# staple/spark-agd

Measured on NVIDIA H100. Metric: AGD examples/sec (rows x applySmooth passes / s), logistic 10M x 1024 dense fp32, higher is better.
Workload: dtype f64

## Files before the change

spark-agd_b200/csrc/k1_tc.cu:

```cuda
#include <cuda.h>
#include <cuda_bf16.h>
#include <cuda_runtime.h>
#include <stdint.h>

#include "agd_common.cuh"
#include "k1_device.cuh"

namespace agd {

namespace {

constexpr int kKR = 16;
constexpr int kRegsConsumer = 64, kRegsAux = 56, kRegsMma = 168;
constexpr int kBlockBytes = kKR * 128;
constexpr int kBBytes = 1024;
constexpr int kScaleOff = 768;

__device__ __forceinline__ uint32_t smem_u32(const void *p) { return (uint32_t)__cvta_generic_to_shared(p); }
__device__ __forceinline__ void mbar_init(uint32_t bar, uint32_t count) {
  asm volatile("mbarrier.init.shared::cta.b64 [%0], %1;" ::"r"(bar), "r"(count));
}
__device__ __forceinline__ void mbar_expect_tx(uint32_t bar, uint32_t bytes) {
  asm volatile("mbarrier.arrive.expect_tx.shared::cta.b64 _, [%0], %1;" ::"r"(bar), "r"(bytes) : "memory");
}
__device__ __forceinline__ void mbar_arrive(uint32_t bar) {
  asm volatile("mbarrier.arrive.shared::cta.b64 _, [%0];" ::"r"(bar) : "memory");
}
__device__ __forceinline__ void mbar_wait(uint32_t bar, uint32_t parity) {
  asm volatile(
      "{\n\t.reg .pred p;\n\t"
      "WAIT_LOOP:\n\t"
      "mbarrier.try_wait.parity.shared::cta.b64 p, [%0], %1;\n\t"
      "@p bra WAIT_DONE;\n\t"
      "bra WAIT_LOOP;\n\t"
      "WAIT_DONE:\n\t}" ::"r"(bar),
      "r"(parity)
      : "memory");
}
__device__ __forceinline__ void named_arrive(int id, int count) {
// ... 1 lines not shown
}
__device__ __forceinline__ void named_sync(int id, int count) {
  asm volatile("bar.sync %0, %1;" ::"r"(id), "r"(count) : "memory");
}
__device__ __forceinline__ void tma_bulk_g2s(uint32_t dst, const void *src, uint32_t bytes, uint32_t bar) {
  asm volatile("cp.async.bulk.shared::cluster.global.mbarrier::complete_tx::bytes [%0], [%1], %2, [%3];" ::"r"(dst),
               "l"(src), "r"(bytes), "r"(bar)
               : "memory");
}
__device__ __forceinline__ void tma_tile_2d(uint32_t dst, const CUtensorMap *map, int c0, int c1, uint32_t bar) {
  asm volatile("cp.async.bulk.tensor.2d.shared::cluster.global.mbarrier::complete_tx::bytes [%0], [%1, {%2, %3}], [%4];" ::"r"(dst),
               "l"(map), "r"(c0), "r"(c1), "r"(bar)
               : "memory");
}
__device__ __forceinline__ void tma_tile_3d(uint32_t dst, const CUtensorMap *map, int c0, int c1, int c2, uint32_t bar) {
  asm volatile("cp.async.bulk.tensor.3d.shared::cluster.global.mbarrier::complete_tx::bytes [%0], [%1, {%2, %3, %4}], [%5];" ::"r"(dst),
               "l"(map), "r"(c0), "r"(c1), "r"(c2), "r"(bar)
               : "memory");
}
__device__ __forceinline__ uint64_t gmma_desc(uint32_t addr, uint32_t lbo, uint32_t sbo, uint64_t layout) {
  return (uint64_t)((addr & 0x3FFFF) >> 4) | ((uint64_t)(lbo >> 4) << 16) | ((uint64_t)(sbo >> 4) << 32) | (layout << 62);
}
__device__ __forceinline__ void wgmma_fence() { asm volatile("wgmma.fence.sync.aligned;" ::: "memory"); }
__device__ __forceinline__ void wgmma_commit() { asm volatile("wgmma.commit_group.sync.aligned;" ::: "memory"); }
template <int N>
__device__ __forceinline__ void wgmma_wait() { asm volatile("wgmma.wait_group.sync.aligned %0;" ::"n"(N) : "memory"); }
template <int N>
__device__ __forceinline__ void wgmma_bf16(float (&d)[N / 2], uint64_t adesc, uint64_t bdesc);
template <>
__device__ __forceinline__ void wgmma_bf16<16>(float (&d)[8], uint64_t adesc, uint64_t bdesc) {
  asm volatile("{ .reg .pred p; setp.ne.b32 p, 0, 0;\n\t"
               "wgmma.mma_async.sync.aligned.m64n16k16.f32.bf16.bf16 {%0,%1,%2,%3,%4,%5,%6,%7}, %8, %9, p, 1, 1, 1, 0; }"
               : "+f"(d[0]), "+f"(d[1]), "+f"(d[2]), "+f"(d[3]), "+f"(d[4]), "+f"(d[5]), "+f"(d[6]), "+f"(d[7])
               : "l"(adesc), "l"(bdesc)
               : "memory");
}
template <>
__device__ __forceinline__ void wgmma_bf16<24>(float (&d)[12], uint64_t adesc, uint64_t bdesc) {
  asm volatile("{ .reg .pred p; setp.ne.b32 p, 0, 0;\n\t"
               "wgmma.mma_async.sync.aligned.m64n24k16.f32.bf16.bf16 {%0,%1,%2,%3,%4,%5,%6,%7,%8,%9,%10,%11}, %12, %13, p, 1, 1, 1, 0; }"
               : "+f"(d[0]), "+f"(d[1]), "+f"(d[2]), "+f"(d[3]), "+f"(d[4]), "+f"(d[5]), "+f"(d[6]), "+f"(d[7]),
                 "+f"(d[8]), "+f"(d[9]), "+f"(d[10]), "+f"(d[11])
               : "l"(adesc), "l"(bdesc)
               : "memory");
}

template <int N, bool TWO>
__device__ __forceinline__ void mma_accumulate(const float (&e)[2][N / 2], int hb, int hs, const double (&sc)[2], double &g,
                                               double *g2) {
  float v[6];
#pragma unroll
  for (int t = 0; t < (TWO ? 6 : 3); ++t) {
    const int i = t == 0 ? 0 : t == 1 ? 1 : t == 2 ? 4 : t == 3 ? 5 : t == 4 ? 8 : 9;
    const float x0 = hs ? e[0][i + 2] : e[0][i], x1 = hs ? e[1][i + 2] : e[1][i];
    v[t] = hb ? x1 : x0;
  }
  g += (((double)v[0] + (double)v[1]) + (double)v[2]) * sc[0];
  if (TWO) *g2 += (((double)v[3] + (double)v[4]) + (double)v[5]) * sc[1];
}
__device__ __forceinline__ double pow2i(int k) { return __longlong_as_double((long long)(k + 1023) << 52); }
__device__ __forceinline__ void mma_release(uint32_t empty_bar, int lane) {
  __syncwarp();
  if (lane == 0) mbar_arrive(empty_bar);
}

struct TcLayout {
  uint32_t ring_off, w_off, b2_off, partial_off, bars_off, g2_off, total;
};
__host__ __device__ inline TcLayout tc_layout(int ring_groups, int group_bytes, int d, bool two_gradient) {
  TcLayout L;
  L.ring_off = 0;
  L.w_off = (uint32_t)ring_groups * group_bytes;
  L.b2_off = L.w_off + (uint32_t)d * 8;
  L.partial_off = L.b2_off + 2 * kBBytes;
  L.bars_off = L.partial_off + 2 * kKR * 16 * 8;
  L.g2_off = L.bars_off + (2 * (uint32_t)ring_groups + 8) * 8;
  L.total = L.g2_off + (two_gradient ? (uint32_t)d * 8 : 0u);
  return L;
}

struct TcArgs {
  const double *labels;
  const double *w;
  const double *w2;
  double *slabs;
  long long rows;
  int d, kind, slab_stride;
  unsigned long long sample_seed, sample_thresh;
  long long row_base;
  const RowFilter *filt;
  const uint32_t *view_bits;
  int gb;
  int ngt;
  int ring_groups;
  int one_copy;
  int diag;
};

__host__ __device__ constexpr int tc_consumers(int rpt) { return rpt == 4 ? 256 : 512; }
__device__ __forceinline__ unsigned long long ffma2(unsigned long long a, unsigned long long b, unsigned long long c) {
  const float x = __fmaf_rn(__uint_as_float((uint32_t)a), __uint_as_float((uint32_t)b), __uint_as_float((uint32_t)c));
  const float y = __fmaf_rn(__uint_as_float((uint32_t)(a >> 32)), __uint_as_float((uint32_t)(b >> 32)),
                            __uint_as_float((uint32_t)(c >> 32)));
  return ((unsigned long long)__float_as_uint(y) << 32) | __float_as_uint(x);
}
__device__ __forceinline__ unsigned long long pack2(uint32_t lo, uint32_t hi) {
  unsigned long long d;
  asm("mov.b64 %0, {%1, %2};" : "=l"(d) : "r"(lo), "r"(hi));
  return d;
}

template <int RPT, bool F32, int DUAL, bool VIEW, bool BIAS>
__global__ void __launch_bounds__(tc_consumers(RPT) + 256, 1)
k1_tc_kernel(const __grid_constant__ CUtensorMap tmap, const __grid_constant__ CUtensorMap tmap3, const TcArgs a,
             const long long ntiles) {
  constexpr int kConsumers = tc_consumers(RPT);
  constexpr int kThreads = kConsumers + 256;
  constexpr int kN = DUAL == 2 ? 24 : 16;
  constexpr int kCW = kConsumers / 32;
  constexpr bool kRepartition = RPT != 4;
  extern __shared__ __align__(1024) unsigned char smem[];
  const int group_bytes = a.gb * kBlockBytes;
  const TcLayout L = tc_layout(a.ring_groups, group_bytes, a.d, DUAL == 2);
  double *w_s = reinterpret_cast<double *>(smem + L.w_off);
  unsigned char *b2 = smem + L.b2_off;
  double *partial = reinterpret_cast<double *>(smem + L.partial_off);
  const uint32_t bars = smem_u32(smem + L.bars_off);
  const int RG = a.ring_groups;
  const uint32_t wbar = bars + 16u * RG, b2_full = wbar + 8, b2_empty = b2_full + 16;
  const int tid = threadIdx.x, warp = tid >> 5, lane = tid & 31;
  const long long my_tiles = (ntiles - blockIdx.x + gridDim.x - 1) / gridDim.x;
  const int npairs = a.d / 128;
  double *slab = a.slabs + (size_t)blockIdx.x * a.slab_stride;

  if (tid == 0) {
    for (int g = 0; g < RG; ++g) {
      mbar_init(bars + 8u * g, 1);
      mbar_init(bars + 8u * (RG + g), 4);
    }
    mbar_init(wbar, 1);
    mbar_init(b2_full, 1); mbar_init(b2_full + 8, 1);
    mbar_init(b2_empty, 4); mbar_init(b2_empty + 8, 4);
    asm volatile("fence.mbarrier_init.release.cluster;" ::: "memory");
  }
  for (int i = tid; i < 2 * kBBytes / 4; i += kThreads) reinterpret_cast<uint32_t *>(b2)[i] = 0u;
  asm volatile("fence.proxy.async.shared::cta;" ::: "memory");
  __syncthreads();

  if (warp >= kCW && warp < kCW + 4) {
   if (kRepartition) asm volatile("setmaxnreg.dec.sync.aligned.u32 %0;" ::"n"(kRegsAux));
   if (warp == kCW) {
    if (lane == 0) {
      mbar_expect_tx(wbar, (uint32_t)a.d * 8u);
      tma_bulk_g2s(smem_u32(w_s), a.w, (uint32_t)a.d * 8u, wbar);
      int slot = -1;
      uint32_t epar = 0;
      bool wrapped = false;
      for (long long k = 0; k < my_tiles; ++k) {
        const long long row0 = (blockIdx.x + k * (long long)gridDim.x) * kKR;
        for (int gi = 0; gi < a.ngt; ++gi) {
          if (++slot == RG) { slot = 0; if (wrapped) epar ^= 1u; wrapped = true; }
          if (wrapped) mbar_wait(bars + 8u * (RG + slot), epar);
          const uint32_t full = bars + 8u * slot;
          mbar_expect_tx(full, (uint32_t)group_bytes);
          if (a.one_copy) {
            tma_tile_3d(smem_u32(smem + (size_t)slot * group_bytes), &tmap3, 0, (int)row0, gi * a.gb, full);
          } else {
            for (int b = 0; b < a.gb; ++b)
              tma_tile_2d(smem_u32(smem + (size_t)slot * group_bytes + b * kBlockBytes), &tmap, (gi * a.gb + b) * 64, (int)row0, full);
          }
        }
      }
    }
   } else if (warp == kCW + 2) {
    double lossacc = 0.0, cntacc = 0.0, multacc = 0.0;
    double ynext = 0.0;
    const int srow = lane & 15;
    const bool second = DUAL && lane >= kKR;
    if (lane < kKR || DUAL) {
      const long long r = (long long)blockIdx.x * kKR + srow;
      if (r < a.rows) ynext = a.labels[r];
    }
    const double *partial2 = partial + 2 * kKR * 2;
    for (long long k = 0; k < my_tiles; ++k) {
      const int bb = (int)(k & 1);
      const long long tile = blockIdx.x + k * (long long)gridDim.x;
      const long long left = a.rows - tile * kKR;
      const int rv = left < kKR ? (int)left : kKR;
      const double ylab = ynext;
      if (lane < kKR || DUAL) {
        const long long r = (tile + gridDim.x) * kKR + srow;
        if (r < a.rows) ynext = a.labels[r];
      }
      named_sync(1 + bb, kConsumers + 32);
      double mult = 0.0;
      bool nonfinite = false;
      if (lane < kKR || second) {
        double m;
        if (RPT) {
          const double *pp = second ? partial2 : partial;
          m = pp[(bb * kKR + srow) * 2] + pp[(bb * kKR + srow) * 2 + 1];
        } else {
          const double *pp = partial + (bb * kKR + lane) * 16;
          m = (((pp[0] + pp[1]) + (pp[2] + pp[3])) + ((pp[4] + pp[5]) + (pp[6] + pp[7]))) +
              (((pp[8] + pp[9]) + (pp[10] + pp[11])) + ((pp[12] + pp[13]) + (pp[14] + pp[15])));
        }
        if (BIAS) m += ld_volatile_f64(second ? a.w2 + a.d : a.w + a.d);
        nonfinite = (lane < kKR || DUAL == 2) && srow < rv && !isfinite(m);
        double mu, loss;
        loss_eval(a.kind, m, ylab, mu, loss);
        if (srow < rv && (!VIEW || ((a.view_bits[(tile * kKR + srow) >> 5] >> ((tile * kKR + srow) & 31)) & 1u) != 0u) &&
            row_selected(a.sample_seed, a.sample_thresh, a.row_base + tile * kKR + srow)) {
          mult = mu; lossacc += loss; cntacc += 1.0;
          if (BIAS) multacc += mu;
        }
      }
      named_arrive(3 + bb, kConsumers + 32);
      const uint32_t hw = (uint32_t)__double2hiint(mult) & 0x7fffffffu;
      const uint32_t hwf = hw | (nonfinite ? 0x80000000u : 0u);
      uint32_t top = __reduce_max_sync(0xffffffffu, lane < kKR ? hwf : 0u), top2 = 0u;
      if (DUAL == 2) top2 = __reduce_max_sync(0xffffffffu, lane < kKR ? 0u : hwf);
      if ((top | top2) >> 31) {
        top = __reduce_max_sync(0xffffffffu, lane < kKR ? hw : 0u);
        if (DUAL == 2) top2 = __reduce_max_sync(0xffffffffu, lane < kKR ? 0u : hw);
        const uint32_t fl = __ballot_sync(0xffffffffu, nonfinite && mult == 0.0);
        const uint32_t zero_rows = DUAL == 2 ? (fl & (fl >> 16) & 0xffffu) : fl;
        const int slot0 = (int)((k * a.ngt) % RG);
#pragma unroll 1
        for (uint32_t rows = zero_rows; rows; rows &= rows - 1u) {
          const int zr = __ffs(rows) - 1;
          int sl = slot0;
#pragma unroll 1
          for (int gi = 0; gi < a.ngt; ++gi) {
#pragma unroll 1
            for (int c = lane; c < a.gb * 8; c += 32)
              *reinterpret_cast<uint4 *>(smem + sl * group_bytes + (c >> 3) * kBlockBytes + zr * 128 + (c & 7) * 16) =
                  make_uint4(0u, 0u, 0u, 0u);
            if (++sl == RG) sl = 0;
          }
        }
      }
      uint32_t E = top >> 20;
      if (DUAL == 2 && second) E = top2 >> 20;
      const int s = E == 0x7ffu ? 0 : E == 0u ? -1022 : E == 0x7feu ? 1023 : (int)E - 1022;
      const int ns = -s;
      const double ms = (mult * pow2i(ns >> 1)) * pow2i(ns - (ns >> 1));
      if (k >= 2) mbar_wait(b2_empty + 8u * bb, (uint32_t)(((k >> 1) - 1) & 1));
      if (srow == 0 && (lane < kKR || (DUAL == 2 && second))) {
        reinterpret_cast<double *>(b2 + bb * kBBytes + kScaleOff)[second ? 1 : 0] = pow2i(s);
      }
      if (lane < kKR || (DUAL == 2 && second)) {
        const __nv_bfloat16 hi = __double2bfloat16(ms);
        const double r1 = ms - (double)__bfloat162float(hi);
        const __nv_bfloat16 mid = __double2bfloat16(r1);
        const double r2 = r1 - (double)__bfloat162float(mid);
        const __nv_bfloat16 lo = __double2bfloat16(r2);
        const int n0 = second ? 9 : 0, n1 = second ? 16 : 1, n2 = second ? 17 : 8;
        unsigned char *base = b2 + bb * kBBytes + (srow / 8) * 128 + (srow % 8) * 2;
#pragma unroll
        for (int t = 0; t < 4; ++t) {
          const int c0 = n0 + 2 * t, c1 = n1 + 2 * t, c2 = n2 + 2 * t;
          *reinterpret_cast<__nv_bfloat16 *>(base + (c0 / 8) * 256 + (c0 % 8) * 16) = hi;
          *reinterpret_cast<__nv_bfloat16 *>(base + (c1 / 8) * 256 + (c1 % 8) * 16) = mid;
          *reinterpret_cast<__nv_bfloat16 *>(base + (c2 / 8) * 256 + (c2 % 8) * 16) = lo;
        }
      }
      asm volatile("fence.proxy.async.shared::cta;" ::: "memory");
      __syncwarp();
      if (lane == 0) mbar_arrive(b2_full + 8u * bb);
    }
    for (int off = DUAL ? 8 : 16; off >= 1; off >>= 1) {
      lossacc += __shfl_xor_sync(0xffffffffu, lossacc, off);
      cntacc += __shfl_xor_sync(0xffffffffu, cntacc, off);
      if (BIAS) multacc += __shfl_xor_sync(0xffffffffu, multacc, off);
    }
    const int DB = a.d + (BIAS ? 1 : 0);
    if (lane == 0) {
      if (BIAS) slab[a.d] = multacc;
      slab[DB] = lossacc; slab[DB + 1] = cntacc; if (!DUAL) { slab[DB + 2] = 0.0; slab[DB + 3] = 0.0; }
    }
    if (DUAL && lane == kKR) {
      slab[DB + 2] = lossacc; slab[DB + 3] = cntacc;
      if (DUAL == 2) {
        double *slab2 = slab + DB + 4;
        if (BIAS) slab2[a.d] = multacc;
        slab2[DB] = lossacc; slab2[DB + 1] = cntacc; slab2[DB + 2] = 0.0; slab2[DB + 3] = 0.0;
      }
    }
   }
  } else if (warp >= kCW + 4) {
    if (kRepartition) asm volatile("setmaxnreg.inc.sync.aligned.u32 %0;" ::"n"(kRegsMma));
    const int mw = warp - (kCW + 4);
    const int q = lane >> 2, j = lane & 3;
    const int hb = j >> 1, hs = j & 1;
    const int fo = 64 * hb + 16 * mw + q + 8 * hs;
    double gacc[32];
#pragma unroll
    for (int p = 0; p < 32; ++p) gacc[p] = 0.0;
    double *g2 = reinterpret_cast<double *>(smem + L.g2_off);
    if (DUAL == 2)
      for (int p = 0; p < npairs; ++p) g2[128 * p + fo] = 0.0;
    const int hp = a.gb / 2;
    int slot = -1;
    uint32_t par = 1;
    float acc[2][kN / 2];
    for (long long k = 0; k < my_tiles; ++k) {
      const int bb = (int)(k & 1);
      mbar_wait(b2_full + 8u * bb, (uint32_t)((k >> 1) & 1));
      const uint64_t bdesc = gmma_desc(smem_u32(b2 + bb * kBBytes), 128, 256, 0);
      const double *scs = reinterpret_cast<const double *>(b2 + bb * kBBytes + kScaleOff);
      const double sc[2] = {scs[0], DUAL == 2 ? scs[1] : 1.0};
#pragma unroll
      for (int p = 0; p < 32; ++p) {
        if (p < npairs) {
          const int pg = p % hp;
          if (pg == 0) {
            if (++slot == RG) slot = 0;
            if (slot == 0) par ^= 1u;
            mbar_wait(bars + 8u * slot, par);
          }
          const uint32_t a0 = smem_u32(smem + (size_t)slot * group_bytes + (2 * pg) * kBlockBytes);
          wgmma_fence();
          if (a.diag != 101) {
            wgmma_bf16<kN>(acc[0], gmma_desc(a0, kBlockBytes, 1024, 1), bdesc);
            wgmma_bf16<kN>(acc[1], gmma_desc(a0 + kBlockBytes, kBlockBytes, 1024, 1), bdesc);
          }
          wgmma_commit();
          wgmma_wait<0>();
          mma_accumulate<kN, DUAL == 2>(acc, hb, hs, sc, gacc[p], g2 + 128 * p + fo);
          if (pg == hp - 1) mma_release(bars + 8u * (RG + slot), lane);
        }
      }
      __syncwarp();
      if (lane == 0) mbar_arrive(b2_empty + 8u * bb);
    }
#pragma unroll
    for (int p = 0; p < 32; ++p)
      if (p < npairs) {
        slab[128 * p + fo] = gacc[p];
        if (DUAL == 2) slab[a.d + (BIAS ? 1 : 0) + 4 + 128 * p + fo] = g2[128 * p + fo];
      }
  } else {
    if (kRepartition) asm volatile("setmaxnreg.dec.sync.aligned.u32 %0;" ::"n"(kRegsConsumer));
    if constexpr (RPT == 0) {
      const int r = lane & 15, hsel = lane >> 4;
      mbar_wait(wbar, 0);
      int slot = -1;
      uint32_t par = 1;
      const int npairs = a.gb * 4;
      uint32_t x_off[2];
      int w_off[2];
      bool act[2];
#pragma unroll
      for (int j = 0; j < 2; ++j) {
        const int c = 2 * (warp + 16 * j) + hsel;
        act[j] = warp + 16 * j < npairs;
        x_off[j] = (uint32_t)((c >> 3) * kBlockBytes + r * 128 + (((c & 7) ^ (r & 7)) << 4));
        w_off[j] = c * 8;
      }
      for (long long k = 0; k < my_tiles; ++k) {
        const int bb = (int)(k & 1);
        double pa[2] = {0.0, 0.0}, pb[2] = {0.0, 0.0};
        const double *wp = w_s;
        for (int gi = 0; gi < a.ngt; ++gi) {
          if (++slot == RG) slot = 0;
          if (slot == 0) par ^= 1u;
          mbar_wait(bars + 8u * slot, par);
          if (a.diag != 100) {
            const unsigned char *gbase = smem + (uint32_t)slot * (uint32_t)group_bytes;
#pragma unroll
            for (int j = 0; j < 2; ++j) {
              if (act[j]) {
                const uint4 xr = *reinterpret_cast<const uint4 *>(gbase + x_off[j]);
                const double2 *wv = reinterpret_cast<const double2 *>(wp + w_off[j]);
#pragma unroll
                for (int q = 0; q < 4; ++q) {
                  const double2 wq = wv[q];
                  const uint32_t xw = q == 0 ? xr.x : q == 1 ? xr.y : q == 2 ? xr.z : xr.w;
                  pa[j] = fma((double)__uint_as_float(xw << 16), wq.x, pa[j]);
                  pb[j] = fma((double)__uint_as_float(xw & 0xffff0000u), wq.y, pb[j]);
                }
              }
            }
          }
          wp += a.gb * 64;
        }
        double p = (pa[0] + pb[0]) + (pa[1] + pb[1]);
        p += __shfl_xor_sync(0xffffffffu, p, 16);
        if (k >= 2) named_sync(3 + bb, kConsumers + 32);
        if (lane < 16) partial[(bb * kKR + r) * 16 + warp] = p;
        named_arrive(1 + bb, kConsumers + 32);
      }
    } else {
    constexpr int kSlots = kKR / (RPT ? RPT : 1);
    const int rq = tid >> 6;
    const int vv = tid & 63;
    mbar_wait(wbar, 0);
    int slot = -1;
    uint32_t par = 1;
    const int blk = vv >> 3, ch = vv & 7;
    const bool active = vv < a.gb * 8;
    uint32_t x_off[RPT];
#pragma unroll
    for (int j = 0; j < RPT; ++j) {
      const int row = rq + j * kSlots;
      x_off[j] = (uint32_t)(blk * kBlockBytes + row * 128 + ((ch ^ (row & 7)) << 4));
    }
    if constexpr (F32) {
      const int nchunks = a.d / 8;
      float4 lo4[2], hi4[2], lo4b[2], hi4b[2];
#pragma unroll
      for (int i = 0; i < 2; ++i) {
        const int c = tid + i * kConsumers;
        if (c < nchunks) {
          const double *src = w_s + (size_t)c * 8;
          lo4[i] = make_float4((float)src[0], (float)src[1], (float)src[2], (float)src[3]);
          hi4[i] = make_float4((float)src[4], (float)src[5], (float)src[6], (float)src[7]);
          if (DUAL) {
            const double *s2 = a.w2 + (size_t)c * 8;
            lo4b[i] = make_float4((float)s2[0], (float)s2[1], (float)s2[2], (float)s2[3]);
            hi4b[i] = make_float4((float)s2[4], (float)s2[5], (float)s2[6], (float)s2[7]);
          }
        }
      }
      named_sync(5, kConsumers);
      float4 *plane0 = reinterpret_cast<float4 *>(w_s), *plane1 = plane0 + nchunks;
      float4 *plane0b = plane1 + nchunks, *plane1b = plane0b + nchunks;
#pragma unroll
      for (int i = 0; i < 2; ++i) {
        const int c = tid + i * kConsumers;
        if (c < nchunks) {
          plane0[c] = lo4[i]; plane1[c] = hi4[i];
          if (DUAL) { plane0b[c] = lo4b[i]; plane1b[c] = hi4b[i]; }
        }
      }
      named_sync(5, kConsumers);
      double *partial2 = partial + 2 * kKR * 2;
      for (long long k = 0; k < my_tiles; ++k) {
        const int bb = (int)(k & 1);
        double pd[RPT], pd2[RPT];
        unsigned long long acc[RPT], acc2[RPT];
#pragma unroll
        for (int j = 0; j < RPT; ++j) { pd[j] = 0.0; acc[j] = 0ull; pd2[j] = 0.0; acc2[j] = 0ull; }
        const ulonglong2 *wp0 = reinterpret_cast<const ulonglong2 *>(plane0) + vv;
        const ulonglong2 *wp1 = reinterpret_cast<const ulonglong2 *>(plane1) + vv;
        const ulonglong2 *wq0 = reinterpret_cast<const ulonglong2 *>(plane0b) + vv;
        const ulonglong2 *wq1 = reinterpret_cast<const ulonglong2 *>(plane1b) + vv;
        for (int gi = 0; gi < a.ngt; ++gi) {
          if (++slot == RG) slot = 0;
          if (slot == 0) par ^= 1u;
          mbar_wait(bars + 8u * slot, par);
          if (active && a.diag != 100) {
            const unsigned char *gbase = smem + (uint32_t)slot * (uint32_t)group_bytes;
            uint4 xr[RPT];
#pragma unroll
            for (int j = 0; j < RPT; ++j) xr[j] = *reinterpret_cast<const uint4 *>(gbase + x_off[j]);
            const ulonglong2 wa = *wp0, wb = *wp1;
            ulonglong2 va = wa, vb = wb;
            if (DUAL) { va = *wq0; vb = *wq1; }
#pragma unroll
            for (int j = 0; j < RPT; ++j) {
              const unsigned long long x0 = pack2(xr[j].x << 16, xr[j].x & 0xffff0000u), x1 = pack2(xr[j].y << 16, xr[j].y & 0xffff0000u),
                                       x2 = pack2(xr[j].z << 16, xr[j].z & 0xffff0000u), x3 = pack2(xr[j].w << 16, xr[j].w & 0xffff0000u);
              acc[j] = ffma2(x0, wa.x, acc[j]);
              acc[j] = ffma2(x1, wa.y, acc[j]);
              acc[j] = ffma2(x2, wb.x, acc[j]);
              acc[j] = ffma2(x3, wb.y, acc[j]);
              if (DUAL) {
                acc2[j] = ffma2(x0, va.x, acc2[j]);
                acc2[j] = ffma2(x1, va.y, acc2[j]);
                acc2[j] = ffma2(x2, vb.x, acc2[j]);
                acc2[j] = ffma2(x3, vb.y, acc2[j]);
              }
            }
          }
          wp0 += a.gb * 8;
          wp1 += a.gb * 8;
          wq0 += a.gb * 8;
          wq1 += a.gb * 8;
          if ((gi & 1) || gi + 1 == a.ngt) {
#pragma unroll
            for (int j = 0; j < RPT; ++j) {
              pd[j] += (double)(__uint_as_float((uint32_t)acc[j]) + __uint_as_float((uint32_t)(acc[j] >> 32)));
              acc[j] = 0ull;
              if (DUAL) {
                pd2[j] += (double)(__uint_as_float((uint32_t)acc2[j]) + __uint_as_float((uint32_t)(acc2[j] >> 32)));
                acc2[j] = 0ull;
              }
            }
          }
        }
        const double tot = warp_rows_reduce<RPT>(pd, lane);
        double tot2 = 0.0;
        if (DUAL) tot2 = warp_rows_reduce<RPT>(pd2, lane);
        if (k >= 2) named_sync(3 + bb, kConsumers + 32);
        if ((lane & (32 / RPT - 1)) == 0) {
          partial[(bb * kKR + rq + kSlots * (lane / (32 / RPT))) * 2 + (warp & 1)] = tot;
          if (DUAL) partial2[(bb * kKR + rq + kSlots * (lane / (32 / RPT))) * 2 + (warp & 1)] = tot2;
        }
        named_arrive(1 + bb, kConsumers + 32);
      }
    } else {
    for (int c = tid; c < a.d / 8; c += kConsumers) {
      const int f = (c >> 1) & 3;
      if (f) {
        double2 *blk = reinterpret_cast<double2 *>(w_s + (size_t)c * 8);
        const double2 t0 = blk[0], t1 = blk[1], t2 = blk[2], t3 = blk[3];
        const double2 v[4] = {t0, t1, t2, t3};
        blk[0 ^ f] = v[0]; blk[1 ^ f] = v[1]; blk[2 ^ f] = v[2]; blk[3 ^ f] = v[3];
      }
    }
    named_sync(5, kConsumers);
    const int sw = (lane >> 1) & 3;
    for (long long k = 0; k < my_tiles; ++k) {
      const int bb = (int)(k & 1);
      double pa[RPT], pb[RPT];
#pragma unroll
      for (int j = 0; j < RPT; ++j) { pa[j] = 0.0; pb[j] = 0.0; }
      const double *wp = w_s + (blk * 64 + ch * 8);
      for (int gi = 0; gi < a.ngt; ++gi) {
        if (++slot == RG) slot = 0;
        if (slot == 0) par ^= 1u;
        mbar_wait(bars + 8u * slot, par);
        if (active && a.diag != 100) {
          const unsigned char *gbase = smem + (uint32_t)slot * (uint32_t)group_bytes;
          uint4 xr[RPT];
#pragma unroll
          for (int j = 0; j < RPT; ++j) xr[j] = *reinterpret_cast<const uint4 *>(gbase + x_off[j]);
#pragma unroll
          for (int q = 0; q < 4; ++q) {
            const double2 wq = *reinterpret_cast<const double2 *>(wp + 2 * (q ^ sw));
#pragma unroll
            for (int j = 0; j < RPT; ++j) {
              const uint32_t xw = q == 0 ? xr[j].x : q == 1 ? xr[j].y : q == 2 ? xr[j].z : xr[j].w;
              pa[j] = fma((double)__uint_as_float(xw << 16), wq.x, pa[j]);
              pb[j] = fma((double)__uint_as_float(xw & 0xffff0000u), wq.y, pb[j]);
            }
          }
        }
        wp += a.gb * 64;
      }
      double p[RPT];
#pragma unroll
      for (int j = 0; j < RPT; ++j) p[j] = pa[j] + pb[j];
      const double tot = warp_rows_reduce<RPT>(p, lane);
      if (k >= 2) named_sync(3 + bb, kConsumers + 32);
      if ((lane & (32 / RPT - 1)) == 0) partial[(bb * kKR + rq + kSlots * (lane / (32 / RPT))) * 2 + (warp & 1)] = tot;
      named_arrive(1 + bb, kConsumers + 32);
    }
    }
    }
  }
}

template <int SITE, typename K>
cudaError_t set_smem_once(K kern, int bytes) {
  static int cur[64] = {0};
  int dev = 0;
  cudaError_t e = cudaGetDevice(&dev);
  if (e != cudaSuccess) return e;
  if (dev >= 0 && dev < 64 && cur[dev] == bytes) return cudaSuccess;
  e = cudaFuncSetAttribute(kern, cudaFuncAttributeMaxDynamicSharedMemorySize, bytes);
  if (e == cudaSuccess && dev >= 0 && dev < 64) cur[dev] = bytes;
  return e;
}

template <bool VIEW, bool BIAS>
cudaError_t tc_launch_forms(const K1Args &a, const CUtensorMap &tmap, const CUtensorMap &tmap3, const TcArgs &t, long long grid,
                            int smem_bytes, long long ntiles, cudaStream_t st) {
  cudaError_t e;
  if (a.tune_rows == 1) {
    e = set_smem_once<1 + 8 * VIEW + 16 * BIAS>(k1_tc_kernel<0, false, 0, VIEW, BIAS>, smem_bytes);
    if (e != cudaSuccess) return e;
    k1_tc_kernel<0, false, 0, VIEW, BIAS><<<(unsigned)grid, 768, smem_bytes, st>>>(tmap, tmap3, t, ntiles);
  } else if (a.tune_rows == 4) {
    e = set_smem_once<2 + 8 * VIEW + 16 * BIAS>(k1_tc_kernel<4, false, 0, VIEW, BIAS>, smem_bytes);
    if (e != cudaSuccess) return e;
    k1_tc_kernel<4, false, 0, VIEW, BIAS><<<(unsigned)grid, 512, smem_bytes, st>>>(tmap, tmap3, t, ntiles);
  } else if (a.tc_margins_f64) {
    e = set_smem_once<3 + 8 * VIEW + 16 * BIAS>(k1_tc_kernel<2, false, 0, VIEW, BIAS>, smem_bytes);
    if (e != cudaSuccess) return e;
    k1_tc_kernel<2, false, 0, VIEW, BIAS><<<(unsigned)grid, 768, smem_bytes, st>>>(tmap, tmap3, t, ntiles);
  } else if (a.w2 && a.dual_full) {
    e = set_smem_once<6 + 8 * VIEW + 16 * BIAS>(k1_tc_kernel<2, true, 2, VIEW, BIAS>, smem_bytes);
    if (e != cudaSuccess) return e;
    k1_tc_kernel<2, true, 2, VIEW, BIAS><<<(unsigned)grid, 768, smem_bytes, st>>>(tmap, tmap3, t, ntiles);
  } else if (a.w2) {
    e = set_smem_once<4 + 8 * VIEW + 16 * BIAS>(k1_tc_kernel<2, true, 1, VIEW, BIAS>, smem_bytes);
    if (e != cudaSuccess) return e;
    k1_tc_kernel<2, true, 1, VIEW, BIAS><<<(unsigned)grid, 768, smem_bytes, st>>>(tmap, tmap3, t, ntiles);
  } else {
    e = set_smem_once<5 + 8 * VIEW + 16 * BIAS>(k1_tc_kernel<2, true, 0, VIEW, BIAS>, smem_bytes);
    if (e != cudaSuccess) return e;
    k1_tc_kernel<2, true, 0, VIEW, BIAS><<<(unsigned)grid, 768, smem_bytes, st>>>(tmap, tmap3, t, ntiles);
  }
  return cudaGetLastError();
}

typedef CUresult (*EncodeTiledFn)(CUtensorMap *, CUtensorMapDataType, cuuint32_t, void *, const cuuint64_t *, const cuuint64_t *,
                                  const cuuint32_t *, const cuuint32_t *, CUtensorMapInterleave, CUtensorMapSwizzle,
                                  CUtensorMapL2promotion, CUtensorMapFloatOOBfill);

}

int k1_tc_supported(int32_t d, int elem_bytes) { return elem_bytes == 2 && d >= 128 && d <= 4096 && d % 128 == 0; }

cudaError_t k1_tc_launch(const K1Args &a, int bias, int sm_count, int *blocks_out, cudaStream_t st) {
  if (!k1_tc_supported(a.d, 2)) return cudaErrorInvalidValue;
  if (a.rows <= 0) { *blocks_out = 0; return cudaSuccess; }
  static EncodeTiledFn encode = nullptr;
  if (!encode) {
    void *fn = nullptr;
    cudaDriverEntryPointQueryResult qres;
    cudaError_t e = cudaGetDriverEntryPoint("cuTensorMapEncodeTiled", &fn, cudaEnableDefault, &qres);
    if (e != cudaSuccess || !fn) return e != cudaSuccess ? e : cudaErrorUnknown;
    encode = (EncodeTiledFn)fn;
  }
  CUtensorMap tmap;
// ... 22 lines not shown
  TcArgs t;
  t.one_copy = a.tune_ctas == 2 ? 0 : 1;
  t.diag = (a.kind == 100 || a.kind == 101) ? a.kind : 0;
  if (a.w2 && (a.tune_rows != 0 || a.tc_margins_f64)) return cudaErrorInvalidValue;
  t.labels = a.labels; t.w = a.w; t.w2 = a.w2; t.slabs = a.slabs; t.rows = a.rows; t.d = a.d; t.kind = a.kind;
  t.slab_stride = a.slab_stride;
  t.sample_seed = a.sample_seed; t.sample_thresh = a.sample_thresh; t.row_base = a.row_base; t.filt = a.filt; t.view_bits = a.view_bits;
  t.gb = gb;
  t.ngt = nblk / gb;
  const int group_bytes = t.gb * kBlockBytes;
  int ring = a.stages > 0 ? a.stages : 16;
  const bool two_gradient = a.w2 && a.dual_full;
  const uint32_t budget = 227u * 1024u - 2048u;
  while (ring > 2 && tc_layout(ring, group_bytes, a.d, two_gradient).total + 1024 > budget) --ring;
  if (ring < t.ngt + 1) ring = t.ngt + 1;
  t.ring_groups = ring;
  const TcLayout L = tc_layout(ring, group_bytes, a.d, two_gradient);
  if (L.total + 1024 > budget) return cudaErrorInvalidValue;
  const long long ntiles = (a.rows + kKR - 1) / kKR;
  long long grid = sm_count;
  if (grid > ntiles) grid = ntiles;
  *blocks_out = (int)grid;
  const int smem_bytes = (int)L.total + 1024;
  if (bias)
    return a.filt ? tc_launch_forms<true, true>(a, tmap, tmap3, t, grid, smem_bytes, ntiles, st)
                  : tc_launch_forms<false, true>(a, tmap, tmap3, t, grid, smem_bytes, ntiles, st);
  return a.filt ? tc_launch_forms<true, false>(a, tmap, tmap3, t, grid, smem_bytes, ntiles, st)
                : tc_launch_forms<false, false>(a, tmap, tmap3, t, grid, smem_bytes, ntiles, st);
}

}
```

Measured before the change: 1.091 billion.

## Software-pipeline wgmma issue across pairs and specialize gradient accumulator count

The MMA warps now issue each pair's wgmma into one of two accumulator sets and wait only for older groups (wait_group 1/2). This lets the tensor-core work for the next pair overlap the fp64 accumulation of the previous one, instead of serializing with wait<0> after every pair. A compile-time NP template (8 for d<=1024, 32 otherwise) shrinks the gacc register array, and register budgets are rebalanced between MMA and aux warps. Ring-slot release is deferred with tracked slots, B/partial buffer counts are parameterized, and optional clock64 profiling is added behind a macro. The added register pressure from two accumulator sets and the more complex release logic carry some risk.

```diff
diff --git a/spark-agd_b200/csrc/k1_tc.cu b/spark-agd_b200/csrc/k1_tc.cu
--- a/spark-agd_b200/csrc/k1_tc.cu
+++ b/spark-agd_b200/csrc/k1_tc.cu
@@ -2,6 +2,11 @@
 #include <cuda_bf16.h>
 #include <cuda_runtime.h>
 #include <stdint.h>
+#ifdef K1_TC_PROFILE
+#include <cstdio>
+#endif
+
+#include <type_traits>
 
 #include "agd_common.cuh"
 #include "k1_device.cuh"
@@ -11,10 +16,12 @@
 namespace {
 
 constexpr int kKR = 16;
-constexpr int kRegsConsumer = 64, kRegsAux = 56, kRegsMma = 168;
+constexpr int kRegsConsumer = 64, kRegsAux = 72, kRegsMma = 152;
 constexpr int kBlockBytes = kKR * 128;
 constexpr int kBBytes = 1024;
 constexpr int kScaleOff = 768;
+constexpr int kBS = 2;
+constexpr int kPartialBytes = kKR * 16 * 8;
 
 __device__ __forceinline__ uint32_t smem_u32(const void *p) { return (uint32_t)__cvta_generic_to_shared(p); }
 __device__ __forceinline__ void mbar_init(uint32_t bar, uint32_t count) {
@@ -62,6 +69,7 @@
   return (uint64_t)((addr & 0x3FFFF) >> 4) | ((uint64_t)(lbo >> 4) << 16) | ((uint64_t)(sbo >> 4) << 32) | (layout << 62);
 }
 __device__ __forceinline__ void wgmma_fence() { asm volatile("wgmma.fence.sync.aligned;" ::: "memory"); }
+__device__ __forceinline__ void wgmma_operand(uint64_t &x) { asm volatile("" : "+l"(x)::"memory"); }
 __device__ __forceinline__ void wgmma_commit() { asm volatile("wgmma.commit_group.sync.aligned;" ::: "memory"); }
 template <int N>
 __device__ __forceinline__ void wgmma_wait() { asm volatile("wgmma.wait_group.sync.aligned %0;" ::"n"(N) : "memory"); }
@@ -69,7 +77,7 @@
 __device__ __forceinline__ void wgmma_bf16(float (&d)[N / 2], uint64_t adesc, uint64_t bdesc);
 template <>
 __device__ __forceinline__ void wgmma_bf16<16>(float (&d)[8], uint64_t adesc, uint64_t bdesc) {
-  asm volatile("{ .reg .pred p; setp.ne.b32 p, 0, 0;\n\t"
+  asm volatile("{ .reg .pred p; setp.ne.b32 p, 1, 0;\n\t"
                "wgmma.mma_async.sync.aligned.m64n16k16.f32.bf16.bf16 {%0,%1,%2,%3,%4,%5,%6,%7}, %8, %9, p, 1, 1, 1, 0; }"
                : "+f"(d[0]), "+f"(d[1]), "+f"(d[2]), "+f"(d[3]), "+f"(d[4]), "+f"(d[5]), "+f"(d[6]), "+f"(d[7])
                : "l"(adesc), "l"(bdesc)
@@ -77,7 +85,7 @@
 }
 template <>
 __device__ __forceinline__ void wgmma_bf16<24>(float (&d)[12], uint64_t adesc, uint64_t bdesc) {
-  asm volatile("{ .reg .pred p; setp.ne.b32 p, 0, 0;\n\t"
+  asm volatile("{ .reg .pred p; setp.ne.b32 p, 1, 0;\n\t"
                "wgmma.mma_async.sync.aligned.m64n24k16.f32.bf16.bf16 {%0,%1,%2,%3,%4,%5,%6,%7,%8,%9,%10,%11}, %12, %13, p, 1, 1, 1, 0; }"
                : "+f"(d[0]), "+f"(d[1]), "+f"(d[2]), "+f"(d[3]), "+f"(d[4]), "+f"(d[5]), "+f"(d[6]), "+f"(d[7]),
                  "+f"(d[8]), "+f"(d[9]), "+f"(d[10]), "+f"(d[11])
@@ -86,8 +94,12 @@
 }
 
 template <int N, bool TWO>
-__device__ __forceinline__ void mma_accumulate(const float (&e)[2][N / 2], int hb, int hs, const double (&sc)[2], double &g,
+__device__ __forceinline__ void mma_accumulate(float (&e)[2][N / 2], int hb, int hs, const double (&sc)[2], double &g,
                                                double *g2) {
+#pragma unroll
+  for (int b = 0; b < 2; ++b)
+#pragma unroll
+    for (int i = 0; i < N / 2; ++i) asm volatile("" : "+f"(e[b][i])::"memory");
   float v[6];
 #pragma unroll
   for (int t = 0; t < (TWO ? 6 : 3); ++t) {
@@ -112,9 +124,9 @@
   L.ring_off = 0;
   L.w_off = (uint32_t)ring_groups * group_bytes;
   L.b2_off = L.w_off + (uint32_t)d * 8;
-  L.partial_off = L.b2_off + 2 * kBBytes;
-  L.bars_off = L.partial_off + 2 * kKR * 16 * 8;
-  L.g2_off = L.bars_off + (2 * (uint32_t)ring_groups + 8) * 8;
+  L.partial_off = L.b2_off + kBS * kBBytes;
+  L.bars_off = L.partial_off + kBS * kPartialBytes;
+  L.g2_off = L.bars_off + (2 * (uint32_t)ring_groups + 1 + 2 * kBS) * 8;
   L.total = L.g2_off + (two_gradient ? (uint32_t)d * 8 : 0u);
   return L;
 }
@@ -137,6 +149,35 @@
   int diag;
 };
 
+#ifdef K1_TC_PROFILE
+__device__ unsigned long long tc_prof[9];
+__global__ void tc_prof_print(int d, long long ntiles) {
+  double v[9];
+  for (int i = 0; i < 9; ++i) {
+    v[i] = (double)tc_prof[i] / (double)ntiles;
+    tc_prof[i] = 0ull;
+  }
+  printf("k1_tc profile d=%d tiles=%lld, cycles per tile: CTA %.0f | producer empty %.0f | consumers full %.0f, "
+         "partial slot %.0f | scalar partials %.0f, B slot %.0f | MMA B %.0f, full %.0f, wgmma_wait %.0f\n",
+         d, ntiles, v[0], v[1], v[2], v[3], v[4], v[5], v[6], v[7], v[8]);
+}
+#define TC_WAIT(i, ...)                      \
+  do {                                       \
+    const long long t0_ = clock64();         \
+    __VA_ARGS__;                             \
+    prof[i] += clock64() - t0_;              \
+  } while (0)
+#else
+#define TC_WAIT(i, ...) __VA_ARGS__
+#endif
+
+__device__ __forceinline__ long long cta_tiles(long long ntiles) {
+  uint32_t b, g;
+  asm volatile("mov.u32 %0, %%ctaid.x;" : "=r"(b));
+  asm volatile("mov.u32 %0, %%nctaid.x;" : "=r"(g));
+  return (ntiles - b + g - 1) / g;
+}
+
 __host__ __device__ constexpr int tc_consumers(int rpt) { return rpt == 4 ? 256 : 512; }
 __device__ __forceinline__ unsigned long long ffma2(unsigned long long a, unsigned long long b, unsigned long long c) {
   const float x = __fmaf_rn(__uint_as_float((uint32_t)a), __uint_as_float((uint32_t)b), __uint_as_float((uint32_t)c));
@@ -150,7 +191,7 @@
   return d;
 }
 
-template <int RPT, bool F32, int DUAL, bool VIEW, bool BIAS>
+template <int RPT, bool F32, int DUAL, bool VIEW, bool BIAS, int NP>
 __global__ void __launch_bounds__(tc_consumers(RPT) + 256, 1)
 k1_tc_kernel(const __grid_constant__ CUtensorMap tmap, const __grid_constant__ CUtensorMap tmap3, const TcArgs a,
              const long long ntiles) {
@@ -165,11 +206,16 @@
   double *w_s = reinterpret_cast<double *>(smem + L.w_off);
   unsigned char *b2 = smem + L.b2_off;
   double *partial = reinterpret_cast<double *>(smem + L.partial_off);
+  double *partial2 = partial + kBS * kKR * 2;
   const uint32_t bars = smem_u32(smem + L.bars_off);
   const int RG = a.ring_groups;
-  const uint32_t wbar = bars + 16u * RG, b2_full = wbar + 8, b2_empty = b2_full + 16;
+  const uint32_t wbar = bars + 16u * RG, b2_full = wbar + 8, b2_empty = b2_full + 8 * kBS;
+  constexpr int kPartFull = 1, kPartFree = 1 + kBS, kConsSync = 1 + 2 * kBS;
   const int tid = threadIdx.x, warp = tid >> 5, lane = tid & 31;
-  const long long my_tiles = (ntiles - blockIdx.x + gridDim.x - 1) / gridDim.x;
+#ifdef K1_TC_PROFILE
+  long long prof[9] = {};
+  if (tid == 0) prof[0] = -clock64();
+#endif
   const int npairs = a.d / 128;
   double *slab = a.slabs + (size_t)blockIdx.x * a.slab_stride;
 
@@ -179,16 +225,19 @@
       mbar_init(bars + 8u * (RG + g), 4);
     }
     mbar_init(wbar, 1);
-    mbar_init(b2_full, 1); mbar_init(b2_full + 8, 1);
-    mbar_init(b2_empty, 4); mbar_init(b2_empty + 8, 4);
+    for (int b = 0; b < kBS; ++b) {
+      mbar_init(b2_full + 8u * b, 1);
+      mbar_init(b2_empty + 8u * b, 4);
+    }
     asm volatile("fence.mbarrier_init.release.cluster;" ::: "memory");
   }
-  for (int i = tid; i < 2 * kBBytes / 4; i += kThreads) reinterpret_cast<uint32_t *>(b2)[i] = 0u;
+  for (int i = tid; i < kBS * kBBytes / 4; i += kThreads) reinterpret_cast<uint32_t *>(b2)[i] = 0u;
   asm volatile("fence.proxy.async.shared::cta;" ::: "memory");
   __syncthreads();
 
   if (warp >= kCW && warp < kCW + 4) {
    if (kRepartition) asm volatile("setmaxnreg.dec.sync.aligned.u32 %0;" ::"n"(kRegsAux));
+   const long long my_tiles = cta_tiles(ntiles);
    if (warp == kCW) {
     if (lane == 0) {
       mbar_expect_tx(wbar, (uint32_t)a.d * 8u);
@@ -200,7 +249,7 @@
         const long long row0 = (blockIdx.x + k * (long long)gridDim.x) * kKR;
         for (int gi = 0; gi < a.ngt; ++gi) {
           if (++slot == RG) { slot = 0; if (wrapped) epar ^= 1u; wrapped = true; }
-          if (wrapped) mbar_wait(bars + 8u * (RG + slot), epar);
+          if (wrapped) TC_WAIT(1, mbar_wait(bars + 8u * (RG + slot), epar));
           const uint32_t full = bars + 8u * slot;
           mbar_expect_tx(full, (uint32_t)group_bytes);
           if (a.one_copy) {
@@ -221,9 +270,8 @@
       const long long r = (long long)blockIdx.x * kKR + srow;
       if (r < a.rows) ynext = a.labels[r];
     }
-    const double *partial2 = partial + 2 * kKR * 2;
     for (long long k = 0; k < my_tiles; ++k) {
-      const int bb = (int)(k & 1);
+      const int bs = (int)(k % kBS);
       const long long tile = blockIdx.x + k * (long long)gridDim.x;
       const long long left = a.rows - tile * kKR;
       const int rv = left < kKR ? (int)left : kKR;
@@ -232,16 +280,16 @@
         const long long r = (tile + gridDim.x) * kKR + srow;
         if (r < a.rows) ynext = a.labels[r];
       }
-      named_sync(1 + bb, kConsumers + 32);
+      TC_WAIT(4, named_sync(kPartFull + bs, kConsumers + 32));
       double mult = 0.0;
       bool nonfinite = false;
       if (lane < kKR || second) {
         double m;
         if (RPT) {
           const double *pp = second ? partial2 : partial;
-          m = pp[(bb * kKR + srow) * 2] + pp[(bb * kKR + srow) * 2 + 1];
+          m = pp[(bs * kKR + srow) * 2] + pp[(bs * kKR + srow) * 2 + 1];
         } else {
-          const double *pp = partial + (bb * kKR + lane) * 16;
+          const double *pp = partial + (bs * kKR + lane) * 16;
           m = (((pp[0] + pp[1]) + (pp[2] + pp[3])) + ((pp[4] + pp[5]) + (pp[6] + pp[7]))) +
               (((pp[8] + pp[9]) + (pp[10] + pp[11])) + ((pp[12] + pp[13]) + (pp[14] + pp[15])));
         }
@@ -255,7 +303,7 @@
           if (BIAS) multacc += mu;
         }
       }
-      named_arrive(3 + bb, kConsumers + 32);
+      named_arrive(kPartFree + bs, kConsumers + 32);
       const uint32_t hw = (uint32_t)__double2hiint(mult) & 0x7fffffffu;
       const uint32_t hwf = hw | (nonfinite ? 0x80000000u : 0u);
       uint32_t top = __reduce_max_sync(0xffffffffu, lane < kKR ? hwf : 0u), top2 = 0u;
@@ -285,9 +333,9 @@
       const int s = E == 0x7ffu ? 0 : E == 0u ? -1022 : E == 0x7feu ? 1023 : (int)E - 1022;
       const int ns = -s;
       const double ms = (mult * pow2i(ns >> 1)) * pow2i(ns - (ns >> 1));
-      if (k >= 2) mbar_wait(b2_empty + 8u * bb, (uint32_t)(((k >> 1) - 1) & 1));
+      if (k >= kBS) TC_WAIT(5, mbar_wait(b2_empty + 8u * bs, (uint32_t)((k / kBS - 1) & 1)));
       if (srow == 0 && (lane < kKR || (DUAL == 2 && second))) {
-        reinterpret_cast<double *>(b2 + bb * kBBytes + kScaleOff)[second ? 1 : 0] = pow2i(s);
+        reinterpret_cast<double *>(b2 + bs * kBBytes + kScaleOff)[second ? 1 : 0] = pow2i(s);
       }
       if (lane < kKR || (DUAL == 2 && second)) {
         const __nv_bfloat16 hi = __double2bfloat16(ms);
@@ -296,7 +344,7 @@
         const double r2 = r1 - (double)__bfloat162float(mid);
         const __nv_bfloat16 lo = __double2bfloat16(r2);
         const int n0 = second ? 9 : 0, n1 = second ? 16 : 1, n2 = second ? 17 : 8;
-        unsigned char *base = b2 + bb * kBBytes + (srow / 8) * 128 + (srow % 8) * 2;
+        unsigned char *base = b2 + bs * kBBytes + (srow / 8) * 128 + (srow % 8) * 2;
 #pragma unroll
         for (int t = 0; t < 4; ++t) {
           const int c0 = n0 + 2 * t, c1 = n1 + 2 * t, c2 = n2 + 2 * t;
@@ -307,7 +355,7 @@
       }
       asm volatile("fence.proxy.async.shared::cta;" ::: "memory");
       __syncwarp();
-      if (lane == 0) mbar_arrive(b2_full + 8u * bb);
+      if (lane == 0) mbar_arrive(b2_full + 8u * bs);
     }
     for (int off = DUAL ? 8 : 16; off >= 1; off >>= 1) {
       lossacc += __shfl_xor_sync(0xffffffffu, lossacc, off);
@@ -330,58 +378,96 @@
    }
   } else if (warp >= kCW + 4) {
     if (kRepartition) asm volatile("setmaxnreg.inc.sync.aligned.u32 %0;" ::"n"(kRegsMma));
+    const long long my_tiles = cta_tiles(ntiles);
     const int mw = warp - (kCW + 4);
     const int q = lane >> 2, j = lane & 3;
     const int hb = j >> 1, hs = j & 1;
     const int fo = 64 * hb + 16 * mw + q + 8 * hs;
-    double gacc[32];
-#pragma unroll
-    for (int p = 0; p < 32; ++p) gacc[p] = 0.0;
+    double gacc[NP];
+#pragma unroll
+    for (int p = 0; p < NP; ++p) gacc[p] = 0.0;
     double *g2 = reinterpret_cast<double *>(smem + L.g2_off);
     if (DUAL == 2)
       for (int p = 0; p < npairs; ++p) g2[128 * p + fo] = 0.0;
     const int hp = a.gb / 2;
     int slot = -1;
     uint32_t par = 1;
-    float acc[2][kN / 2];
-    for (long long k = 0; k < my_tiles; ++k) {
-      const int bb = (int)(k & 1);
-      mbar_wait(b2_full + 8u * bb, (uint32_t)((k >> 1) & 1));
-      const uint64_t bdesc = gmma_desc(smem_u32(b2 + bb * kBBytes), 128, 256, 0);
-      const double *scs = reinterpret_cast<const double *>(b2 + bb * kBBytes + kScaleOff);
-      const double sc[2] = {scs[0], DUAL == 2 ? scs[1] : 1.0};
-#pragma unroll
-      for (int p = 0; p < 32; ++p) {
-        if (p < npairs) {
-          const int pg = p % hp;
-          if (pg == 0) {
-            if (++slot == RG) slot = 0;
-            if (slot == 0) par ^= 1u;
-            mbar_wait(bars + 8u * slot, par);
+    constexpr bool kPad = DUAL != 2;
+    constexpr int kSets = 2;
+    float acc[kSets][2][kN / 2];
+    auto tiles = [&](auto issue) {
+      constexpr bool kIssue = decltype(issue)::value;
+      for (long long k = 0; k < my_tiles; ++k) {
+        const int bs = (int)(k % kBS);
+        TC_WAIT(6, mbar_wait(b2_full + 8u * bs, (uint32_t)((k / kBS) & 1)));
+        uint64_t bdesc = gmma_desc(smem_u32(b2 + bs * kBBytes), 128, 256, 0);
+        wgmma_operand(bdesc);
+        const double *scs = reinterpret_cast<const double *>(b2 + bs * kBBytes + kScaleOff);
+        const double sc[2] = {scs[0], DUAL == 2 ? scs[1] : 1.0};
+        int pg = hp - 1, fg = hp - 1;
+        uint32_t a0 = 0;
+        int qslot[kSets];
+#pragma unroll
+        for (int p = 0; p < NP + kSets - 1; ++p) {
+          if (p < NP && (kPad || p < npairs)) {
+            if (p < npairs) {
+              if (++pg == hp) {
+                pg = 0;
+                if (++slot == RG) slot = 0;
+                if (slot == 0) par ^= 1u;
+                TC_WAIT(7, mbar_wait(bars + 8u * slot, par));
+              }
+              a0 = smem_u32(smem + (size_t)slot * group_bytes + (2 * pg) * kBlockBytes);
+            }
+            qslot[p % kSets] = slot;
+            if constexpr (kIssue) {
+              uint64_t ad0 = gmma_desc(a0, kBlockBytes, 1024, 1), ad1 = gmma_desc(a0 + kBlockBytes, kBlockBytes, 1024, 1);
+              wgmma_operand(ad0);
+              wgmma_operand(ad1);
+#pragma unroll
+              for (int b = 0; b < 2; ++b)
+#pragma unroll
+                for (int i = 0; i < kN / 2; ++i) {
+                  acc[p % kSets][b][i] = 0.f;
+                  asm volatile("" : "+f"(acc[p % kSets][b][i])::"memory");
+                }
+              wgmma_fence();
+              wgmma_bf16<kN>(acc[p % kSets][0], ad0, bdesc);
+              wgmma_bf16<kN>(acc[p % kSets][1], ad1, bdesc);
+              wgmma_commit();
+            }
           }
-          const uint32_t a0 = smem_u32(smem + (size_t)slot * group_bytes + (2 * pg) * kBlockBytes);
-          wgmma_fence();
-          if (a.diag != 101) {
-            wgmma_bf16<kN>(acc[0], gmma_desc(a0, kBlockBytes, 1024, 1), bdesc);
-            wgmma_bf16<kN>(acc[1], gmma_desc(a0 + kBlockBytes, kBlockBytes, 1024, 1), bdesc);
+          const int q = p - (kSets - 1);
+          if (q >= 0) {
+            if constexpr (kIssue) {
+              const int later = kPad ? (p < NP ? p : NP - 1) - q : 0;
+              if (later >= 2) TC_WAIT(8, wgmma_wait<2>());
+              else if (later == 1) TC_WAIT(8, wgmma_wait<1>());
+              else TC_WAIT(8, wgmma_wait<0>());
+            }
+            if (q < npairs) {
+              if constexpr (kIssue)
+                mma_accumulate<kN, DUAL == 2>(acc[q % kSets], hb, hs, sc, gacc[q], g2 + 128 * q + fo);
+              if (++fg == hp) fg = 0;
+              if (fg == hp - 1 && q < npairs - 1) mma_release(bars + 8u * (RG + qslot[q % kSets]), lane);
+            }
           }
-          wgmma_commit();
-          wgmma_wait<0>();
-          mma_accumulate<kN, DUAL == 2>(acc, hb, hs, sc, gacc[p], g2 + 128 * p + fo);
-          if (pg == hp - 1) mma_release(bars + 8u * (RG + slot), lane);
-        }
-      }
-      __syncwarp();
-      if (lane == 0) mbar_arrive(b2_empty + 8u * bb);
-    }
-#pragma unroll
-    for (int p = 0; p < 32; ++p)
+        }
+        mma_release(bars + 8u * (RG + slot), lane);
+        __syncwarp();
+        if (lane == 0) mbar_arrive(b2_empty + 8u * bs);
+      }
+    };
+    if (a.diag == 101) tiles(std::false_type{}); else tiles(std::true_type{});
+#pragma unroll
+    for (int p = 0; p < NP; ++p)
       if (p < npairs) {
         slab[128 * p + fo] = gacc[p];
         if (DUAL == 2) slab[a.d + (BIAS ? 1 : 0) + 4 + 128 * p + fo] = g2[128 * p + fo];
       }
   } else {
     if (kRepartition) asm volatile("setmaxnreg.dec.sync.aligned.u32 %0;" ::"n"(kRegsConsumer));
+    const long long my_tiles = cta_tiles(ntiles);
     if constexpr (RPT == 0) {
       const int r = lane & 15, hsel = lane >> 4;
       mbar_wait(wbar, 0);
@@ -399,7 +485,7 @@
         w_off[j] = c * 8;
       }
       for (long long k = 0; k < my_tiles; ++k) {
-        const int bb = (int)(k & 1);
+        const int bs = (int)(k % kBS);
         double pa[2] = {0.0, 0.0}, pb[2] = {0.0, 0.0};
         const double *wp = w_s;
         for (int gi = 0; gi < a.ngt; ++gi) {
@@ -427,9 +513,9 @@
         }
         double p = (pa[0] + pb[0]) + (pa[1] + pb[1]);
         p += __shfl_xor_sync(0xffffffffu, p, 16);
-        if (k >= 2) named_sync(3 + bb, kConsumers + 32);
-        if (lane < 16) partial[(bb * kKR + r) * 16 + warp] = p;
-        named_arrive(1 + bb, kConsumers + 32);
+        if (k >= kBS) named_sync(kPartFree + bs, kConsumers + 32);
+        if (lane < 16) partial[(bs * kKR + r) * 16 + warp] = p;
+        named_arrive(kPartFull + bs, kConsumers + 32);
       }
     } else {
     constexpr int kSlots = kKR / (RPT ? RPT : 1);
@@ -463,7 +549,7 @@
           }
         }
       }
-      named_sync(5, kConsumers);
+      named_sync(kConsSync, kConsumers);
       float4 *plane0 = reinterpret_cast<float4 *>(w_s), *plane1 = plane0 + nchunks;
       float4 *plane0b = plane1 + nchunks, *plane1b = plane0b + nchunks;
 #pragma unroll
@@ -474,10 +560,9 @@
           if (DUAL) { plane0b[c] = lo4b[i]; plane1b[c] = hi4b[i]; }
         }
       }
-      named_sync(5, kConsumers);
-      double *partial2 = partial + 2 * kKR * 2;
+      named_sync(kConsSync, kConsumers);
       for (long long k = 0; k < my_tiles; ++k) {
-        const int bb = (int)(k & 1);
+        const int bs = (int)(k % kBS);
         double pd[RPT], pd2[RPT];
         unsigned long long acc[RPT], acc2[RPT];
 #pragma unroll
@@ -489,7 +574,7 @@
         for (int gi = 0; gi < a.ngt; ++gi) {
           if (++slot == RG) slot = 0;
           if (slot == 0) par ^= 1u;
-          mbar_wait(bars + 8u * slot, par);
+          TC_WAIT(2, mbar_wait(bars + 8u * slot, par));
           if (active && a.diag != 100) {
             const unsigned char *gbase = smem + (uint32_t)slot * (uint32_t)group_bytes;
             uint4 xr[RPT];
@@ -533,12 +618,12 @@
         const double tot = warp_rows_reduce<RPT>(pd, lane);
         double tot2 = 0.0;
         if (DUAL) tot2 = warp_rows_reduce<RPT>(pd2, lane);
-        if (k >= 2) named_sync(3 + bb, kConsumers + 32);
+        if (k >= kBS) TC_WAIT(3, named_sync(kPartFree + bs, kConsumers + 32));
         if ((lane & (32 / RPT - 1)) == 0) {
-          partial[(bb * kKR + rq + kSlots * (lane / (32 / RPT))) * 2 + (warp & 1)] = tot;
-          if (DUAL) partial2[(bb * kKR + rq + kSlots * (lane / (32 / RPT))) * 2 + (warp & 1)] = tot2;
-        }
-        named_arrive(1 + bb, kConsumers + 32);
+          partial[(bs * kKR + rq + kSlots * (lane / (32 / RPT))) * 2 + (warp & 1)] = tot;
+          if (DUAL) partial2[(bs * kKR + rq + kSlots * (lane / (32 / RPT))) * 2 + (warp & 1)] = tot2;
+        }
+        named_arrive(kPartFull + bs, kConsumers + 32);
       }
     } else {
     for (int c = tid; c < a.d / 8; c += kConsumers) {
@@ -550,10 +635,10 @@
         blk[0 ^ f] = v[0]; blk[1 ^ f] = v[1]; blk[2 ^ f] = v[2]; blk[3 ^ f] = v[3];
       }
     }
-    named_sync(5, kConsumers);
+    named_sync(kConsSync, kConsumers);
     const int sw = (lane >> 1) & 3;
     for (long long k = 0; k < my_tiles; ++k) {
-      const int bb = (int)(k & 1);
+      const int bs = (int)(k % kBS);
       double pa[RPT], pb[RPT];
 #pragma unroll
       for (int j = 0; j < RPT; ++j) { pa[j] = 0.0; pb[j] = 0.0; }
@@ -584,13 +669,19 @@
 #pragma unroll
       for (int j = 0; j < RPT; ++j) p[j] = pa[j] + pb[j];
       const double tot = warp_rows_reduce<RPT>(p, lane);
-      if (k >= 2) named_sync(3 + bb, kConsumers + 32);
-      if ((lane & (32 / RPT - 1)) == 0) partial[(bb * kKR + rq + kSlots * (lane / (32 / RPT))) * 2 + (warp & 1)] = tot;
-      named_arrive(1 + bb, kConsumers + 32);
+      if (k >= kBS) named_sync(kPartFree + bs, kConsumers + 32);
+      if ((lane & (32 / RPT - 1)) == 0) partial[(bs * kKR + rq + kSlots * (lane / (32 / RPT))) * 2 + (warp & 1)] = tot;
+      named_arrive(kPartFull + bs, kConsumers + 32);
     }
     }
     }
   }
+#ifdef K1_TC_PROFILE
+  if (tid == 0) prof[0] += clock64();
+  if (tid == 0 || ((warp == kCW || warp == kCW + 2 || warp == kCW + 4) && lane == 0))
+    for (int i = 0; i < 9; ++i)
+      if (prof[i]) atomicAdd(&tc_prof[i], (unsigned long long)prof[i]);
+#endif
 }
 
 template <int SITE, typename K>
@@ -605,35 +696,38 @@
   return e;
 }
 
-template <bool VIEW, bool BIAS>
+template <bool VIEW, bool BIAS, int NP>
 cudaError_t tc_launch_forms(const K1Args &a, const CUtensorMap &tmap, const CUtensorMap &tmap3, const TcArgs &t, long long grid,
                             int smem_bytes, long long ntiles, cudaStream_t st) {
   cudaError_t e;
   if (a.tune_rows == 1) {
-    e = set_smem_once<1 + 8 * VIEW + 16 * BIAS>(k1_tc_kernel<0, false, 0, VIEW, BIAS>, smem_bytes);
+    e = set_smem_once<1 + 8 * VIEW + 16 * BIAS + 32 * (NP > 8)>(k1_tc_kernel<0, false, 0, VIEW, BIAS, NP>, smem_bytes);
     if (e != cudaSuccess) return e;
-    k1_tc_kernel<0, false, 0, VIEW, BIAS><<<(unsigned)grid, 768, smem_bytes, st>>>(tmap, tmap3, t, ntiles);
+    k1_tc_kernel<0, false, 0, VIEW, BIAS, NP><<<(unsigned)grid, 768, smem_bytes, st>>>(tmap, tmap3, t, ntiles);
   } else if (a.tune_rows == 4) {
-    e = set_smem_once<2 + 8 * VIEW + 16 * BIAS>(k1_tc_kernel<4, false, 0, VIEW, BIAS>, smem_bytes);
+    e = set_smem_once<2 + 8 * VIEW + 16 * BIAS + 32 * (NP > 8)>(k1_tc_kernel<4, false, 0, VIEW, BIAS, NP>, smem_bytes);
     if (e != cudaSuccess) return e;
-    k1_tc_kernel<4, false, 0, VIEW, BIAS><<<(unsigned)grid, 512, smem_bytes, st>>>(tmap, tmap3, t, ntiles);
+    k1_tc_kernel<4, false, 0, VIEW, BIAS, NP><<<(unsigned)grid, 512, smem_bytes, st>>>(tmap, tmap3, t, ntiles);
   } else if (a.tc_margins_f64) {
-    e = set_smem_once<3 + 8 * VIEW + 16 * BIAS>(k1_tc_kernel<2, false, 0, VIEW, BIAS>, smem_bytes);
+    e = set_smem_once<3 + 8 * VIEW + 16 * BIAS + 32 * (NP > 8)>(k1_tc_kernel<2, false, 0, VIEW, BIAS, NP>, smem_bytes);
     if (e != cudaSuccess) return e;
-    k1_tc_kernel<2, false, 0, VIEW, BIAS><<<(unsigned)grid, 768, smem_bytes, st>>>(tmap, tmap3, t, ntiles);
+    k1_tc_kernel<2, false, 0, VIEW, BIAS, NP><<<(unsigned)grid, 768, smem_bytes, st>>>(tmap, tmap3, t, ntiles);
   } else if (a.w2 && a.dual_full) {
-    e = set_smem_once<6 + 8 * VIEW + 16 * BIAS>(k1_tc_kernel<2, true, 2, VIEW, BIAS>, smem_bytes);
+    e = set_smem_once<6 + 8 * VIEW + 16 * BIAS + 32 * (NP > 8)>(k1_tc_kernel<2, true, 2, VIEW, BIAS, NP>, smem_bytes);
     if (e != cudaSuccess) return e;
-    k1_tc_kernel<2, true, 2, VIEW, BIAS><<<(unsigned)grid, 768, smem_bytes, st>>>(tmap, tmap3, t, ntiles);
+    k1_tc_kernel<2, true, 2, VIEW, BIAS, NP><<<(unsigned)grid, 768, smem_bytes, st>>>(tmap, tmap3, t, ntiles);
   } else if (a.w2) {
-    e = set_smem_once<4 + 8 * VIEW + 16 * BIAS>(k1_tc_kernel<2, true, 1, VIEW, BIAS>, smem_bytes);
+    e = set_smem_once<4 + 8 * VIEW + 16 * BIAS + 32 * (NP > 8)>(k1_tc_kernel<2, true, 1, VIEW, BIAS, NP>, smem_bytes);
     if (e != cudaSuccess) return e;
-    k1_tc_kernel<2, true, 1, VIEW, BIAS><<<(unsigned)grid, 768, smem_bytes, st>>>(tmap, tmap3, t, ntiles);
+    k1_tc_kernel<2, true, 1, VIEW, BIAS, NP><<<(unsigned)grid, 768, smem_bytes, st>>>(tmap, tmap3, t, ntiles);
   } else {
-    e = set_smem_once<5 + 8 * VIEW + 16 * BIAS>(k1_tc_kernel<2, true, 0, VIEW, BIAS>, smem_bytes);
+    e = set_smem_once<5 + 8 * VIEW + 16 * BIAS + 32 * (NP > 8)>(k1_tc_kernel<2, true, 0, VIEW, BIAS, NP>, smem_bytes);
     if (e != cudaSuccess) return e;
-    k1_tc_kernel<2, true, 0, VIEW, BIAS><<<(unsigned)grid, 768, smem_bytes, st>>>(tmap, tmap3, t, ntiles);
+    k1_tc_kernel<2, true, 0, VIEW, BIAS, NP><<<(unsigned)grid, 768, smem_bytes, st>>>(tmap, tmap3, t, ntiles);
   }
+#ifdef K1_TC_PROFILE
+  tc_prof_print<<<1, 1, 0, st>>>(a.d, ntiles);
+#endif
   return cudaGetLastError();
 }
 
@@ -702,11 +796,18 @@
   if (grid > ntiles) grid = ntiles;
   *blocks_out = (int)grid;
   const int smem_bytes = (int)L.total + 1024;
+  if (a.d <= 8 * 128) {
+    if (bias)
+      return a.filt ? tc_launch_forms<true, true, 8>(a, tmap, tmap3, t, grid, smem_bytes, ntiles, st)
+                    : tc_launch_forms<false, true, 8>(a, tmap, tmap3, t, grid, smem_bytes, ntiles, st);
+    return a.filt ? tc_launch_forms<true, false, 8>(a, tmap, tmap3, t, grid, smem_bytes, ntiles, st)
+                  : tc_launch_forms<false, false, 8>(a, tmap, tmap3, t, grid, smem_bytes, ntiles, st);
+  }
   if (bias)
-    return a.filt ? tc_launch_forms<true, true>(a, tmap, tmap3, t, grid, smem_bytes, ntiles, st)
-                  : tc_launch_forms<false, true>(a, tmap, tmap3, t, grid, smem_bytes, ntiles, st);
-  return a.filt ? tc_launch_forms<true, false>(a, tmap, tmap3, t, grid, smem_bytes, ntiles, st)
-                : tc_launch_forms<false, false>(a, tmap, tmap3, t, grid, smem_bytes, ntiles, st);
-}
-
-}
+    return a.filt ? tc_launch_forms<true, true, 32>(a, tmap, tmap3, t, grid, smem_bytes, ntiles, st)
+                  : tc_launch_forms<false, true, 32>(a, tmap, tmap3, t, grid, smem_bytes, ntiles, st);
+  return a.filt ? tc_launch_forms<true, false, 32>(a, tmap, tmap3, t, grid, smem_bytes, ntiles, st)
+                : tc_launch_forms<false, false, 32>(a, tmap, tmap3, t, grid, smem_bytes, ntiles, st);
+}
+
+}
```

Measured after the change: 1.091 billion (median of 6 runs). No clear change (-0.0%).
